# sevagh/umx.cpp

Hardware: AMD Instinct MI355X
Metric: realtime-factor (audio-sec/wall-sec) UMX-L 4-stem, 60 s seg (higher is better)
Workload: dtype f32 (activations as 2 x fp16 planes of the power-of-two-scaled row, integer weights exact in fp16, f32 accumulate on the fp16 matrix cores; fp32-grade: 1.4-2.2x the error of an fp32 evaluation, profiles/r06_v2_accuracy_vs_float64.txt)

## Files before the change

umx.cpp_amd/csrc/engine.hip:

```cpp
#include "../../include/umx_hip.h"
#include <chrono>
#include <dlfcn.h>

#include <algorithm>
#include <numeric>
#include <cmath>
#include <cstdio>
#include <cstdlib>
#include <cstring>
#include <map>
#include <mutex>
#include <string>
#include <vector>

#include "common.h"
#include "gemm_bf16x3.h"
#include "gemm_planes.h"
#include "gemm_planes_pp.h"
#include "gemm_planes_ps.h"
#include "lstm_kernels.h"
#include "lstm_batch.h"
#include "lstm_batch8.h"
#include "track_kernels.h"
#include "resample.h"
// ... 273 lines not shown
    int last = 0;
    for (const LstmKernel &k : kLstmKernels)
        if (k.family == family && k.hl != last)
        {
            s += (s.empty() ? "{" : ", ") + std::to_string(2 * k.hl);
            last = k.hl;
        }
    return s + "}";
}

struct GemmKernel
{
    const void *fn = nullptr;
    int lds = 0;
};

template <int MODE> static GemmKernel bx_kernel_m(int bq)
{
    if (bq == BQ_F32)
        return {kernel_ptr(gemm_bf16x3_kernel<MODE, BQ_F32>), BX_LDS_BYTES};
    if constexpr (MODE == G_FC1 || MODE == G_IH)
    {
        if (bq == BQ_U8X)
            return {kernel_ptr(gemm_bf16x3_kernel<MODE, BQ_U8X>), BX_LDS_BYTES};
        if (bq == BQ_U8)
            return {kernel_ptr(gemm_bf16x3_kernel<MODE, BQ_U8>), BX_LDS_BYTES};
    }
    else if (bq == BQ_U16)
        return {kernel_ptr(gemm_bf16x3_kernel<MODE, BQ_U16>), BX_LDS_BYTES};
    return {};
}
static GemmKernel bx_kernel(int mode, int bq)
{
    switch (mode)
    {
    case G_FC1: return bx_kernel_m<G_FC1>(bq);
    case G_IH: return bx_kernel_m<G_IH>(bq);
    case G_FC2: return bx_kernel_m<G_FC2>(bq);
    default: return bx_kernel_m<G_FC3>(bq);
    }
}

enum { GP_128 = 0, GP_256, GP_PP, GP_PS, GP_KINDS };
template <int MODE, int NBP> static GemmKernel gp_kernel_mn(int kind)
{
    switch (kind)
    {
    case GP_128: return {kernel_ptr(gemm_planes_kernel<MODE, NBP, 2, 2>), gp_lds_bytes(2, 2, NBP)};
    case GP_256: return {kernel_ptr(gemm_planes_kernel<MODE, NBP, 4, 4>), gp_lds_bytes(4, 4, NBP)};
    case GP_PP: return {kernel_ptr(gemm_planes_pp_kernel<MODE, NBP>), gp_lds_bytes(4, 4, NBP)};
    default: return {kernel_ptr(gemm_planes_ps_kernel<MODE, NBP>), ps_lds_bytes(NBP)};
    }
}
template <int MODE> static GemmKernel gp_kernel_m(int nbp, int kind)
{
    if constexpr (MODE == G_FC1 || MODE == G_IH)
    {
        if (nbp == 1)
            return gp_kernel_mn<MODE, 1>(kind);
    }
    return nbp == 2 ? gp_kernel_mn<MODE, 2>(kind) : GemmKernel{};
}
static GemmKernel gp_kernel(int mode, int nbp, int kind)
{
    switch (mode)
    {
    case G_FC1: return gp_kernel_m<G_FC1>(nbp, kind);
    case G_IH: return gp_kernel_m<G_IH>(nbp, kind);
    case G_FC2: return gp_kernel_m<G_FC2>(nbp, kind);
    default: return gp_kernel_m<G_FC3>(nbp, kind);
    }
}

struct umx_hip_ctx
{
    int device = 0, H = 0, Hl = 0, S = 0, N = 0, T = 0, Tp = 0, nbatch = 0;
    static constexpr int Mpad = 256;
    std::string err;
    std::vector<void *> allocs;
    TargetBufs tb[4];
    float *whh[3] = {}, *bhh[3] = {};
    float *window = nullptr, *nw = nullptr;
    float2 *tw1 = nullptr, *tw2 = nullptr;
    float *tap_tmp = nullptr;
    float *audio_in = nullptr, *out_dev[4] = {};
    static constexpr int kMaxSlots = 3;
    float *stage_in[kMaxSlots] = {}, *stage_out[kMaxSlots][4 * LSTMB_MAX_TRACKS] = {};
    int ensure_staging();
    hipEvent_t order_ev = nullptr;
    struct DeferredDownload
    {
        bool valid = false;
        int si = 0, nb = 0, n[LSTMB_MAX_TRACKS] = {};
        float *host[4 * LSTMB_MAX_TRACKS] = {};
    };
    int queue_download(const DeferredDownload &d, hipStream_t on);
    hipStream_t copy_stream = nullptr;
    float *state = nullptr, *state_alt = nullptr;
    Slot slot[kMaxSlots];
    int nslots = 2;
    int next_slot() const { return (int)(nseg % nslots); }
    void clear_used()
    {
        for (int si = 0; si < kMaxSlots; ++si)
            slot[si].used = false;
    }
    int B = 1;
    bool lstm_batched = false;
    unsigned tag_epoch = 0;
    unsigned next_tag_base()
    {
        tag_epoch = (tag_epoch + 1) & 0xFFFFF;
        return tag_epoch << 12;
    }
    int cur = 0;
    long long nseg = 0;
    size_t lsync_words = 0;
    bool persistent_ok = true;
    int n_cus = 256;
    struct PendingCall
    {
        int nb;
        const float *audio[LSTMB_MAX_TRACKS];
        int n[LSTMB_MAX_TRACKS];
        float *out[4 * LSTMB_MAX_TRACKS];
        float *host_out[4 * LSTMB_MAX_TRACKS];
        const float *host_audio[LSTMB_MAX_TRACKS];
        unsigned flags;
    };
    static constexpr int kBackupCalls = 8;
    std::vector<PendingCall> pending;
    bool pending_lost = false;
    float *backup = nullptr;
    bool no_recovery = false, recovering = false;
    int recover();
    int lstm_poll_delay = 0;
    int env_gemm_ps = -1;
    int env_gemm_pp = -1;
    const char *gemm_kernel_last[4] = {"none", "none", "none", "none"};
    const char *lstm_kernel_last = "none";
    int lstm_capacity = 0;
    unsigned last_flags = 0;
    hipStream_t stream = nullptr;

    void set_error(const std::string &s) { err = s; }

    template <class T_> int dalloc(T_ **p, size_t count, bool zero = true)
    {
        void *q = nullptr;
        UMX_HIP_CHECK(hipMalloc(&q, std::max<size_t>(count, 1) * sizeof(T_)));
        allocs.push_back(q);
        if (zero)
            UMX_HIP_CHECK(hipMemset(q, 0, std::max<size_t>(count, 1) * sizeof(T_)));
        *p = reinterpret_cast<T_ *>(q);
        return UMX_OK;
    }
    template <class T_> int upload(T_ **p, const std::vector<T_> &h)
    {
        int rc = dalloc(p, h.size(), false);
        if (rc)
            return rc;
        UMX_HIP_CHECK(hipMemcpy(*p, h.data(), h.size() * sizeof(T_), hipMemcpyHostToDevice));
        return UMX_OK;
    }
    int init(int device_, int hidden, int segment_samples, const umx_tensor_view *tensors, int n_tensors,
             unsigned create_flags, int n_tracks);
// ... 112 lines not shown
```

umx.cpp_amd/csrc/engine_init.h:

```cpp
namespace
{
bool dequant(const umx_tensor_view &tv, size_t expect, std::vector<float> &out)
{
    size_t nel = 1;
    for (int i = 0; i < tv.n_dims; ++i)
        nel *= (size_t)tv.ne[i];
    if (nel != expect)
        return false;
    out.resize(nel);
    if (tv.dtype == UMX_DTYPE_F32)
        memcpy(out.data(), tv.data, nel * sizeof(float));
    else if (tv.dtype == UMX_DTYPE_U8)
    {
        const uint8_t *q = static_cast<const uint8_t *>(tv.data);
        for (size_t i = 0; i < nel; ++i)
            out[i] = (float)q[i] * tv.scale + tv.offset;
    }
    else if (tv.dtype == UMX_DTYPE_U16)
    {
        const uint16_t *q = static_cast<const uint16_t *>(tv.data);
        for (size_t i = 0; i < nel; ++i)
            out[i] = (float)q[i] * tv.scale + tv.offset;
    }
    else
// ... 312 lines not shown
                std::vector<float> whhv, bih, bhhv;
                if ((!whh_all_u8 && !get(tg, "lstm.weight_hh" + sfx, (size_t)G * Hl, whhv)) ||
                    !get(tg, "lstm.bias_ih" + sfx, G, bih) || !get(tg, "lstm.bias_hh" + sfx, G, bhhv))
                    return UMX_ERR_MODEL;
                const int chain = tg * 2 + dir;
                const umx_tensor_view *hhv = view(tg, "lstm.weight_hh" + sfx);
                const unsigned char *hhq = whh_all_u8 ? static_cast<const unsigned char *>(hhv->data) : nullptr;
                if (whh_all_u8)
                {
                    whh_s[l][chain] = hhv->scale;
                    whh_o[l][chain] = hhv->offset;
                }
                for (int row = 0; row < G; ++row)
                {
                    const int sl = gate_row[row] / 64, col = gate_row[row] % 64;
                    ihb[(size_t)dir * G + gate_row[row]] = bih[row];
                    bhh_h[l][((size_t)chain * S + sl) * 64 + col] = bhhv[row];
                    for (int k = 0; k < Hl; ++k)
                    {
                        const size_t di = (((size_t)chain * S + sl) * Hl + k) * 64 + col;
                        if (whh_all_u8)
                            whh_qh[l][di] = hhq[(size_t)row * Hl + k];
                        else
                            whh_h[l][di] = whhv[(size_t)row * Hl + k];
                    }
                }
            }
            if (int rc = upload(&b.ih_b[l], ihb))
                return rc;
        }
    }
    for (int l = 0; l < 3; ++l)
    {
        if (whh_all_u8)
        {
            if (int rc = upload(&whh_q[l], whh_qh[l]))
                return rc;
            weight_bytes += whh_qh[l].size();
        }
        else
        {
            if (int rc = upload(&whh[l], whh_h[l]))
                return rc;
            weight_bytes += whh_h[l].size() * sizeof(float);
        }
        if (int rc = upload(&bhh[l], bhh_h[l]))
            return rc;
    }
    {
        std::vector<float> w(NFFT);
        static const float PI = 3.14159265359F;
        const float floatN = (float)(NFFT + 1);
        for (int n = 0; n < NFFT; ++n)
            w[n] = 0.5F * (1.0F - cosf(2.0F * PI * (float)n / (floatN - 1)));
        if (int rc = upload(&window, w))
            return rc;
        const size_t total = (size_t)NFFT + (size_t)HOP * (T - 1);
        std::vector<float> nwh(total, 0.f);
        for (int i = 0; i < T; ++i)
        {
            const size_t s0 = (size_t)i * HOP;
            for (size_t j = s0; j < std::min(total, s0 + NFFT); ++j)
                nwh[j] += w[j - s0] * w[j - s0];
        }
        if (int rc = upload(&nw, nwh))
            return rc;
        std::vector<float2> t1(256), t2(4096);
        for (int r = 0; r < 16; ++r)
            for (int k = 0; k < 16; ++k)
            {
                const double ph = -2.0 * M_PI * (double)(r * k) / 256.0;
                t1[r * 16 + k] = make_float2((float)cos(ph), (float)sin(ph));
            }
        for (int r = 0; r < 16; ++r)
            for (int j = 0; j < 256; ++j)
            {
                const double ph = -2.0 * M_PI * (double)(r * j) / 4096.0;
                t2[r * 256 + j] = make_float2((float)cos(ph), (float)sin(ph));
            }
        if (int rc = upload(&tw1, t1))
            return rc;
        if (int rc = upload(&tw2, t2))
            return rc;
    }
    if (int rc = dalloc(&audio_in, (size_t)2 * N))
        return rc;
    for (int k = 0; k < 4; ++k)
        if (int rc = dalloc(&out_dev[k], (size_t)2 * N))
            return rc;
    if (int rc = dalloc(&state, state_floats() * B))
        return rc;
    if (int rc = dalloc(&state_alt, state_floats() * B))
        return rc;
    if (int rc = dalloc(&backup, (size_t)kBackupCalls * 3 * state_floats() * B))
        return rc;
    lsync_words = LSTM_SYNC_HEADER_WORDS + std::max(granule_count(S) * 2, lstm_batched ? lstmb_granule_words(Hl) * ((B + LSTMB_GROUP_TRACKS - 1) / LSTMB_GROUP_TRACKS) : (size_t)0);
    nslots = 2;
    if (gemm_planes)
    {
        const unsigned long long rows = (unsigned long long)B * Tp + Mpad;
        const unsigned long long planes_bytes = 2ull * rows * (unsigned long long)std::max(KX, 2 * H) * 2ull;
        const unsigned long long mask_bytes = (unsigned long long)B * 2ull * T * MAGP * 4ull;
        if (planes_bytes >= (1ull << 31) || mask_bytes >= (1ull << 32))
        {
            set_error("track lanes x segment length exceed the 32-bit addressing of the plane GEMMs' operands: fewer lanes or a shorter segment");
            return UMX_ERR_ARG;
        }
    }
    for (int si = 0; si < nslots; ++si)
    {
        Slot &sl = slot[si];
        UMX_HIP_CHECK(hipStreamCreateWithFlags(&sl.stream, hipStreamNonBlocking));
        float *x_all = nullptr;
        if (int rc = dalloc(&x_all, ((size_t)B * Tp + Mpad) * KX))
            return rc;
        for (int tg = 0; tg < 4; ++tg)
        {
            float *cat_all = nullptr, *la_all = nullptr, *lb_all = nullptr, *P_all = nullptr, *a2_all = nullptr, *mag_all = nullptr;
            if (int rc = dalloc(&cat_all, ((size_t)B * Tp + Mpad) * 2 * H))
                return rc;
            if (int rc = dalloc(&la_all, ((size_t)B * Tp + Mpad) * H))
                return rc;
            if (int rc = dalloc(&lb_all, ((size_t)B * Tp + Mpad) * H))
                return rc;
            if (int rc = dalloc(&P_all, ((size_t)B * Tp + Mpad) * 4 * H))
                return rc;
            if (int rc = dalloc(&a2_all, ((size_t)B * Tp + Mpad) * H))
                return rc;
            if (int rc = dalloc(&mag_all, (size_t)B * 2 * T * MAGP))
                return rc;
            unsigned short *xs_p = nullptr, *cat_p = nullptr, *la_p = nullptr, *lb_p = nullptr, *a2_p = nullptr;
            float *rs[8] = {};
            if (gemm_planes)
            {
                if (int rc = dalloc(&xs_p, 2 * ((size_t)B * Tp + Mpad) * KX))
                    return rc;
                if (int rc = dalloc(&cat_p, 2 * ((size_t)B * Tp + Mpad) * 2 * H))
                    return rc;
                for (unsigned short **q : {&la_p, &lb_p, &a2_p})
                    if (int rc = dalloc(q, 2 * ((size_t)B * Tp + Mpad) * H))
                        return rc;
                for (int k = 0; k < 8; ++k)
                    if (int rc = dalloc(&rs[k], ((size_t)B * Tp + Mpad) * (k >= 2 && k <= 4 ? 2 : 1)))
                        return rc;
            }
            for (int ln = 0; ln < B; ++ln)
            {
                TargetAct &b = sl.lane[ln].ta[tg];
                b.cat = cat_all + (size_t)ln * Tp * 2 * H;
                b.la = la_all + (size_t)ln * Tp * H;
                b.lb = lb_all + (size_t)ln * Tp * H;
                b.P = P_all + (size_t)ln * Tp * 4 * H;
                b.a2 = a2_all + (size_t)ln * Tp * H;
                b.mag = mag_all + (size_t)ln * 2 * T * MAGP;
                if (gemm_planes)
                {
                    b.xs_p = xs_p + (size_t)ln * Tp * KX;
                    b.cat_p = cat_p + (size_t)ln * Tp * 2 * H;
                    b.la_p = la_p + (size_t)ln * Tp * H;
                    b.lb_p = lb_p + (size_t)ln * Tp * H;
                    b.a2_p = a2_p + (size_t)ln * Tp * H;
                    b.rs_xs = rs[0] + (size_t)ln * Tp;
                    b.rs_catL = rs[1] + (size_t)ln * Tp;
                    b.rs_catR = rs[2] + (size_t)ln * Tp;
                    b.rs_la = rs[3] + (size_t)ln * Tp;
                    b.rs_lb = rs[4] + (size_t)ln * Tp;
// ... 146 lines not shown
```

umx.cpp_amd/csrc/engine_stages.h:

```cpp
void umx_hip_ctx::launch_gemm(Lane &sl, hipStream_t st, int mode, int layer, const int *active, int nact, bool dbg)
{
    GemmArgs g;
    memset(&g, 0, sizeof g);
    g.M = Tp;
    g.T = T;
    int bq = BQ_F32;
    for (int i = 0; i < nact; ++i)
    {
        const TargetBufs &b = tb[active[i]];
        const TargetAct &c = sl.ta[active[i]];
        const GemmWeight &w = b.w[gemm_weight(mode, layer)];
        GemmTarget &t = g.t[i];
        switch (mode)
        {
        case G_FC1:
            t.A = sl.x; t.C = c.cat;
            t.e0 = b.bn1[0]; t.e1 = b.bn1[1]; t.e2 = b.bn1[2]; t.e3 = b.bn1[3];
            t.q0 = b.in_scale; t.q1 = b.in_mean;
            g.N = H; g.K = KX; g.lda = KX; g.ldc = 2 * H;
            break;
        case G_IH:
            t.A = layer == 0 ? c.cat : layer == 1 ? c.la : c.lb;
            t.C = c.P; t.e0 = b.ih_b[layer];
            g.N = 4 * H; g.K = H; g.lda = layer == 0 ? 2 * H : H; g.ldc = 4 * H;
// ... 306 lines not shown
        wm0.m[s] = L0.ta[s].mag;
    const int nchunk = (T + WIENER_CHUNK - 1) / WIENER_CHUNK;
    const int iters = (flags & UMX_FLAG_NO_WIENER) ? 1 : std::max(1, (int)((flags & UMX_FLAG_WIENER_ITERS_MASK) >> 16));
    if (iters > 1 && !sl.wv)
    {
        if ((unsigned long long)ls.v * sizeof(float) >= (1ull << 31))
        {
            set_error("Wiener EM iterations: the segment's PSD state exceeds the 32-bit addressing of the filter kernel: a shorter segment");
            return UMX_ERR_ARG;
        }
        if (int rc = dalloc(&sl.wv, (size_t)B * ls.v, false))
            return rc;
    }
    if (flags & UMX_FLAG_NO_WIENER)
    {
        if (!wiener_fused)
            for (int i = 0; i < lanes.count; ++i)
            {
                Lane &L = sl.lane[lanes.id[i]];
                WienerMags wm;
                for (int s = 0; s < 4; ++s)
                    wm.m[s] = L.ta[s].mag;
                const size_t nel = (size_t)2 * T * NBINS;
                hipLaunchKernelGGL(mixphase_kernel, dim3((unsigned)((nel + 255) / 256)), dim3(256), 0, st, L.spec, wm, T, L.y);
            }
    }
    else
    {
        hipLaunchKernelGGL(wiener_stats4_kernel<WIENER_STATS_NS>, dim3((NBINS + 63) / 64, nchunk * lanes.count, 4 / WIENER_STATS_NS), dim3(64), 0, st, L0.spec, wm0, T, L0.maxabs, L0.wpart, lanes, ls);
        hipLaunchKernelGGL(wiener_finish4_kernel, dim3(bt, 4, lanes.count), dim3(256), 0, st, L0.wpart, T, L0.Rc, lanes, ls);
        for (int it = 1; it < iters; ++it)
        {
            if (it == 1)
                hipLaunchKernelGGL(wiener_em_step_kernel<true>, dim3((NBINS + 63) / 64, nchunk * lanes.count), dim3(64), 0, st, L0.spec, wm0, sl.wv, T, L0.maxabs, L0.Rc, L0.wpart, lanes, ls);
            else
                hipLaunchKernelGGL(wiener_em_step_kernel<false>, dim3((NBINS + 63) / 64, nchunk * lanes.count), dim3(64), 0, st, L0.spec, wm0, sl.wv, T, L0.maxabs, L0.Rc, L0.wpart, lanes, ls);
            hipLaunchKernelGGL(wiener_finish4_kernel, dim3(bt, 4, lanes.count), dim3(256), 0, st, L0.wpart, T, L0.Rc, lanes, ls);
        }
        if (!wiener_fused)
            for (int i = 0; i < lanes.count; ++i)
            {
                const int ln = lanes.id[i];
                Lane &L = sl.lane[ln];
                WienerMags wm;
                for (int s = 0; s < 4; ++s)
                    wm.m[s] = L.ta[s].mag;
                if (iters > 1)
                    hipLaunchKernelGGL(wiener_apply_kernel<true>, dim3(bt, T), dim3(256), 0, st, L.spec, wm,
                                       reinterpret_cast<const float4 *>(sl.wv + (size_t)ln * ls.v), T, L.maxabs, L.Rc, L.y);
                else
                    hipLaunchKernelGGL(wiener_apply_kernel<false>, dim3(bt, T), dim3(256), 0, st, L.spec, wm, (const float4 *)nullptr, T, L.maxabs, L.Rc, L.y);
            }
    }
    OlaOut oo;
    oo.lanes = lanes;
    int nmax = 1;
    for (int i = 0; i < lanes.count; ++i)
    {
        const int ln = lanes.id[i];
        for (int s = 0; s < 4; ++s)
            oo.p[i][s] = out[4 * ln + s];
        oo.n[i] = n[ln];
        nmax = std::max(nmax, n[ln]);
    }
    stage_range(ST_ISTFT);
    UMX_HIP_CHECK(hipEventRecord(sl.ev[ST_ISTFT], st));
    if (!wiener_fused)
    {
        for (int i = 0; i < lanes.count; ++i)
        {
            Lane &L = sl.lane[lanes.id[i]];
            hipLaunchKernelGGL(istft_frames_kernel, dim3(T, 4), dim3(256), 0, st, L.y, T, window, nw, tw1, tw2, L.frames);
        }
    }
    else
    {
        float2 *ydbg = dbg ? L0.y : nullptr;
        if (sl.out_free_valid)
            UMX_HIP_CHECK(hipStreamWaitEvent(st, sl.out_free, 0));
        const int runs = std::max(1, std::min(T / 8, (4 * n_cus + lanes.count - 1) / lanes.count));
        const int run_len = std::max(3, (T + runs - 1) / runs), nruns = (T + run_len - 1) / run_len;
        if (flags & UMX_FLAG_NO_WIENER)
            hipLaunchKernelGGL((wiener_istft_kernel<false>), dim3(nruns, 1, lanes.count), dim3(1024), WI_LDS_BYTES, st, L0.spec, wm0,
                               T, L0.maxabs, L0.Rc, window, nw, tw1, tw2, L0.frames, ydbg, ls, run_len, oo);
        else if (iters > 1)
            hipLaunchKernelGGL(wiener_istft_v_kernel, dim3(nruns, 1, lanes.count), dim3(1024), WI_LDS_BYTES, st, (const float *)sl.wv, L0.spec, wm0,
                               T, L0.maxabs, L0.Rc, window, nw, tw1, tw2, L0.frames, ydbg, ls, run_len, oo);
        else
            hipLaunchKernelGGL((wiener_istft_kernel<true>), dim3(nruns, 1, lanes.count), dim3(1024), WI_LDS_BYTES, st, L0.spec, wm0,
                               T, L0.maxabs, L0.Rc, window, nw, tw1, tw2, L0.frames, ydbg, ls, run_len, oo);
        stage_range(ST_OLA);
        UMX_HIP_CHECK(hipEventRecord(sl.ev[ST_OLA], st));
        hipLaunchKernelGGL(wiener_ola_edges_kernel, dim3(3 * HOP / 256, nruns * 4, lanes.count), dim3(256), 0, st, L0.frames, ls.frames, T, run_len, oo);
    }
    if (!wiener_fused)
    {
        stage_range(ST_OLA);
        UMX_HIP_CHECK(hipEventRecord(sl.ev[ST_OLA], st));
        if (sl.out_free_valid)
            UMX_HIP_CHECK(hipStreamWaitEvent(st, sl.out_free, 0));
        hipLaunchKernelGGL(istft_ola_kernel, dim3((nmax + 255) / 256, 4, lanes.count), dim3(256), 0, st, L0.frames, ls.frames, T, oo);
    }
    stage_range(-1);
    UMX_HIP_CHECK(hipEventRecord(sl.ev[ST_COUNT], st));
    UMX_HIP_CHECK(hipGetLastError());
    sl.have_times = true;
    return UMX_OK;
}

int umx_hip_ctx::infer_device(const float *audio_dev, int n, float *const out[4], unsigned flags)
{
    if (!audio_dev)
    {
        set_error("infer_segment: need 1 <= n <= segment_samples and non-null audio");
        return UMX_ERR_ARG;
    }
    return infer_batch(1, &audio_dev, &n, out, flags);
}

int umx_hip_ctx::infer_batch(int nb, const float *const *audio_dev, const int *n, float *const *out, unsigned flags)
{
    StageRangeCloser close_ranges_on_return;
    if (nb < 1 || nb > B || !audio_dev || !n || !out)
    {
        set_error("infer: need 1 <= n_tracks <= the context's track count and non-null argument arrays");
        return UMX_ERR_ARG;
    }
    if (int rc = check_flags(flags))
        return rc;
    unsigned long long lane_mask = 0;
    for (int ln = 0; ln < nb; ++ln)
    {
        if (!audio_dev[ln])
            continue;
        if (n[ln] < 1 || n[ln] > N)
        {
            set_error("infer_segment: need 1 <= n <= segment_samples and non-null audio");
            return UMX_ERR_ARG;
        }
        for (int s = 0; s < 4; ++s)
            if (!out[4 * ln + s])
            {
                set_error("infer_segment: null output pointer");
                return UMX_ERR_ARG;
            }
        lane_mask |= 1ull << ln;
    }
    if (!lane_mask)
    {
        set_error("infer: no active track lane");
        return UMX_ERR_ARG;
    }
    if (ph_next != -1)
    {
        set_error("infer_segment: a phased segment is open (umx_hip_segment_end first)");
        return UMX_ERR_ARG;
    }
    UMX_HIP_CHECK(hipSetDevice(device));
    const int si = next_slot();
    Slot &sl = slot[si];
    Slot &prev = slot[(si + nslots - 1) % nslots];
    hipStream_t st = sl.stream;
    int active[4], nact;
    active_list(flags, active, nact);
    last_flags = flags;
    const size_t call_idx = pending_lost ? (size_t)kBackupCalls : pending.size();
    if (call_idx >= (size_t)kBackupCalls)
    {
        pending_lost = true;
        pending.clear();
    }
    else
    {
// ... 46 lines not shown
```

umx.cpp_amd/csrc/fft4096.h:

```cpp
#pragma once
#include "common.h"

namespace umx
{

constexpr int FFT_LDS_ELEMS = NFFT + NFFT / 16;

__device__ __forceinline__ int fft_pad(int i) { return i + (i >> 4); }

__device__ __forceinline__ float2 cmul(float2 a, float2 b)
{
    return make_float2(a.x * b.x - a.y * b.y, a.x * b.y + a.y * b.x);
}
__device__ __forceinline__ float2 cmul_tw(float2 a, float2 b)
{
    return make_float2(fmaf(a.x, b.x, -(a.y * b.y)), fmaf(a.x, b.y, a.y * b.x));
}
__device__ __forceinline__ float2 cadd(float2 a, float2 b) { return make_float2(a.x + b.x, a.y + b.y); }
__device__ __forceinline__ float2 csub(float2 a, float2 b) { return make_float2(a.x - b.x, a.y - b.y); }
__device__ __forceinline__ float2 cconj(float2 a) { return make_float2(a.x, -a.y); }

template <bool INV> __device__ __forceinline__ float2 mul_w4(float2 a)
{
    return INV ? make_float2(-a.y, a.x) : make_float2(a.y, -a.x);
}

template <bool INV> __device__ __forceinline__ void fft16(float2 (&v)[16])
{
    constexpr float C1 = 0.92387953251128674f;
    constexpr float S1 = 0.38268343236508977f;
    constexpr float R2 = 0.70710678118654752f;
    constexpr float SG = INV ? 1.0f : -1.0f;
    float2 a[4][4];
#pragma unroll
    for (int r0 = 0; r0 < 4; ++r0)
    {
        float2 x0 = v[r0], x1 = v[4 + r0], x2 = v[8 + r0], x3 = v[12 + r0];
        float2 s02 = cadd(x0, x2), d02 = csub(x0, x2), s13 = cadd(x1, x3), d13 = csub(x1, x3);
        float2 rot = mul_w4<INV>(d13);
        a[r0][0] = cadd(s02, s13);
        a[r0][1] = cadd(d02, rot);
        a[r0][2] = csub(s02, s13);
        a[r0][3] = csub(d02, rot);
    }
    const float2 w1 = make_float2(C1, SG * S1), w2 = make_float2(R2, SG * R2),
                 w3 = make_float2(S1, SG * C1), w6 = make_float2(-R2, SG * R2),
                 w9 = make_float2(-C1, -SG * S1);
    a[1][1] = cmul_tw(a[1][1], w1);
    a[1][2] = cmul_tw(a[1][2], w2);
    a[1][3] = cmul_tw(a[1][3], w3);
    a[2][1] = cmul_tw(a[2][1], w2);
    a[2][2] = mul_w4<INV>(a[2][2]);
    a[2][3] = cmul_tw(a[2][3], w6);
    a[3][1] = cmul_tw(a[3][1], w3);
    a[3][2] = cmul_tw(a[3][2], w6);
    a[3][3] = cmul_tw(a[3][3], w9);
#pragma unroll
    for (int q0 = 0; q0 < 4; ++q0)
    {
        float2 x0 = a[0][q0], x1 = a[1][q0], x2 = a[2][q0], x3 = a[3][q0];
        float2 s02 = cadd(x0, x2), d02 = csub(x0, x2), s13 = cadd(x1, x3), d13 = csub(x1, x3);
        float2 rot = mul_w4<INV>(d13);
        v[q0] = cadd(s02, s13);
        v[4 + q0] = cadd(d02, rot);
        v[8 + q0] = csub(s02, s13);
        v[12 + q0] = csub(d02, rot);
    }
}

template <bool INV, bool KEEP = false>
__device__ __forceinline__ void fft4096(float2 (&v)[16], float2 *buf, const float2 *__restrict__ tw1,
                                        const float2 *__restrict__ tw2, int j)
{
    fft16<INV>(v);
#pragma unroll
    for (int q = 0; q < 16; ++q)
        buf[fft_pad((j << 4) + q)] = v[q];
    __syncthreads();
    {
        const int k = j & 15;
#pragma unroll
        for (int r = 0; r < 16; ++r)
            v[r] = buf[fft_pad(j + 256 * r)];
        __syncthreads();
#pragma unroll
        for (int r = 1; r < 16; ++r)
        {
            float2 w = tw1[r * 16 + k];
            v[r] = cmul_tw(v[r], INV ? cconj(w) : w);
        }
        fft16<INV>(v);
        const int base = ((j - k) << 4) + k;
#pragma unroll
        for (int q = 0; q < 16; ++q)
            buf[fft_pad(base + 16 * q)] = v[q];
    }
    float2 w2[16];
#pragma unroll
    for (int r = 1; r < 16; ++r)
        w2[r] = tw2[r * 256 + j];
    __syncthreads();
    {
#pragma unroll
        for (int r = 0; r < 16; ++r)
            v[r] = buf[fft_pad(j + 256 * r)];
#pragma unroll
        for (int r = 1; r < 16; ++r)
        {
            const float2 w = w2[r];
            v[r] = cmul_tw(v[r], INV ? cconj(w) : w);
        }
        fft16<INV>(v);
        if (!KEEP)
#pragma unroll
            for (int q = 0; q < 16; ++q)
                buf[fft_pad(j + 256 * q)] = v[q];
    }
    if (!KEEP)
        __syncthreads();
}

template <bool INV>
__device__ __forceinline__ void fft4096(float2 (&v)[16], float2 *buf, const float2 *__restrict__ tw1,
                                        const float2 *__restrict__ tw2)
{
    fft4096<INV>(v, buf, tw1, tw2, (int)threadIdx.x);
}

}
```

umx.cpp_amd/csrc/wiener_istft.h:

```cpp
#pragma once
#include "stft_kernels.h"
#include "wiener_kernels.h"

#ifndef WI_PROFILE
#define WI_PROFILE 0
#endif

namespace umx
{

constexpr size_t WI_LDS_BYTES = (size_t)4 * FFT_LDS_ELEMS * sizeof(float2) + NFFT * sizeof(float) + HOP * sizeof(float) + 256 * sizeof(float2);

typedef float wi_f2 __attribute__((ext_vector_type(2)));
__device__ __forceinline__ float2 ld_stream(const float2 *p)
{
    const wi_f2 v = __builtin_nontemporal_load(reinterpret_cast<const wi_f2 *>(p));
    return make_float2(v.x, v.y);
}
__device__ __forceinline__ float ld_stream(const float *p) { return __builtin_nontemporal_load(p); }

typedef unsigned wi_u2 __attribute__((ext_vector_type(2)));
typedef unsigned wi_u4 __attribute__((ext_vector_type(4)));
template <int AUX> __device__ __forceinline__ float2 bld2(__amdgpu_buffer_rsrc_t rs, int voff, int soff)
{
    const wi_u2 v = __builtin_amdgcn_raw_buffer_load_b64(rs, voff, soff, AUX);
    return make_float2(__uint_as_float(v.x), __uint_as_float(v.y));
}
template <int AUX> __device__ __forceinline__ float bld1(__amdgpu_buffer_rsrc_t rs, int voff, int soff)
{
    return __uint_as_float(__builtin_amdgcn_raw_buffer_load_b32(rs, voff, soff, AUX));
}
template <int AUX> __device__ __forceinline__ float4 bld4(__amdgpu_buffer_rsrc_t rs, int voff, int soff)
{
    const wi_u4 v = __builtin_amdgcn_raw_buffer_load_b128(rs, voff, soff, AUX);
    return make_float4(__uint_as_float(v.x), __uint_as_float(v.y), __uint_as_float(v.z), __uint_as_float(v.w));
}
__device__ __forceinline__ void bst2(__amdgpu_buffer_rsrc_t rs, int voff, int soff, float2 v)
{
    const wi_u2 t = {__float_as_uint(v.x), __float_as_uint(v.y)};
    __builtin_amdgcn_raw_buffer_store_b64(t, rs, voff, soff, 0);
}

template <bool WIENER, bool VIN>
__device__ __forceinline__ void wiener_istft_run(const float2 *__restrict__ spec, WienerMags mags, const float *__restrict__ v, int T,
                                                                  const unsigned *__restrict__ maxabs_bits,
                                                                  const float *__restrict__ Rc, const float *__restrict__ window,
                                                                  const float *__restrict__ nw, const float2 *__restrict__ tw1,
                                                                  const float2 *__restrict__ tw2, float2 *__restrict__ frames,
                                                                  float2 *__restrict__ y_dbg, WienerStrides ls, int run_len, OlaOut out)
{
    static_assert(WIENER || !VIN, "the PSDs of the filter");
    extern __shared__ __attribute__((aligned(16))) float2 wi_buf[];
    float *const wi_win = reinterpret_cast<float *>(wi_buf + 4 * FFT_LDS_ELEMS);
    float *const wi_nwp = wi_win + NFFT;
    float2 *const wi_tw1 = reinterpret_cast<float2 *>(wi_nwp + HOP);
    constexpr int NSRC = 4, WI_THREADS = 256 * NSRC;
    const LaneSet &lanes = out.lanes;
    {
        const int ln = lanes.id[blockIdx.z];
        spec += (size_t)ln * ls.spec;
        Rc += (size_t)ln * ls.rc;
        frames += (size_t)ln * ls.frames;
        maxabs_bits += ln;
        if (y_dbg)
            y_dbg += (size_t)ln * ls.y;
        if (VIN)
            v += (size_t)ln * ls.v;
#pragma unroll
        for (int s = 0; s < 4; ++s)
            mags.m[s] += (size_t)ln * ls.mag;
    }
    constexpr int src0 = 0;
    const int tid = threadIdx.x;
#pragma unroll
    for (int r = 0; r < 4; ++r)
        wi_win[tid + 1024 * r] = window[tid + 1024 * r];
    wi_nwp[tid] = nw[3 * HOP + tid];
    if (tid < 256)
        wi_tw1[tid] = tw1[tid];
    const __amdgpu_buffer_rsrc_t rs_spec = __builtin_amdgcn_make_buffer_rsrc(const_cast<float2 *>(spec), 0, (int)((size_t)2 * T * NBINS * 8), 0x00020000);
    __amdgpu_buffer_rsrc_t rs_mag[4];
#pragma unroll
    for (int s = 0; s < 4; ++s)
        rs_mag[s] = __builtin_amdgcn_make_buffer_rsrc(const_cast<float *>(mags.m[s]), 0, (int)((size_t)2 * T * MAGP * 4), 0x00020000);
    const __amdgpu_buffer_rsrc_t rs_v = __builtin_amdgcn_make_buffer_rsrc(const_cast<float *>(v), 0, (int)((size_t)T * NBINS * 16), 0x00020000);
    const __amdgpu_buffer_rsrc_t rs_rc = __builtin_amdgcn_make_buffer_rsrc(const_cast<float *>(Rc), 0, (int)((size_t)4 * NBINS * 16), 0x00020000);
    const __amdgpu_buffer_rsrc_t rs_nw = __builtin_amdgcn_make_buffer_rsrc(const_cast<float *>(nw), 0, (int)(((size_t)(T - 1) * HOP + NFFT) * 4), 0x00020000);
    const float max_abs = WIENER ? wiener_max_abs(maxabs_bits) : 1.0f, rmax = 1.0f / max_abs;
    const int f0 = (int)blockIdx.x * run_len, f1 = min(T, f0 + run_len);
    const int g = __builtin_amdgcn_readfirstlane(tid >> 8);
    float2 *const stem = reinterpret_cast<float2 *>(out.p[blockIdx.z][src0 + g]);
    const int n_out = out.n[blockIdx.z];
    const __amdgpu_buffer_rsrc_t rs_stem = __builtin_amdgcn_make_buffer_rsrc(stem, 0, n_out * 8, 0x00020000);
    [[maybe_unused]] long long pf[5] = {0, 0, 0, 0, 0};
    float2 open[3][4];
#pragma unroll
    for (int c = 0; c < 3; ++c)
#pragma unroll
        for (int q = 0; q < 4; ++q)
            open[c][q] = make_float2(0.f, 0.f);
    float2 Xq[2][2];
    float mq[2][2][4];
#define WI_REQUEST(f_, tl_, q_)                                                                                                        \
    {                                                                                                                                  \
        Xq[q_][0] = bld2<2>(rs_spec, (tl_) * 8, ((0 * T + (f_)) * NBINS + WI_THREADS * (q_)) * 8);                                      \
        Xq[q_][1] = bld2<2>(rs_spec, (tl_) * 8, ((1 * T + (f_)) * NBINS + WI_THREADS * (q_)) * 8);                                      \
        if (VIN)                                                                                                                       \
        {                                                                                                                              \
            const float4 vf_ = bld4<2>(rs_v, (tl_) * 16, ((f_) * NBINS + WI_THREADS * (q_)) * 16);                                      \
            mq[q_][0][0] = vf_.x;                                                                                                      \
            mq[q_][0][1] = vf_.y;                                                                                                      \
            mq[q_][0][2] = vf_.z;                                                                                                      \
            mq[q_][0][3] = vf_.w;                                                                                                      \
        }                                                                                                                              \
        else                                                                                                                           \
            _Pragma("unroll") for (int s = 0; s < 4; ++s)                                                                              \
            {                                                                                                                          \
                mq[q_][0][s] = bld1<2>(rs_mag[s], (tl_) * 4, ((0 * T + (f_)) * MAGP + WI_THREADS * (q_)) * 4);  \
                mq[q_][1][s] = bld1<2>(rs_mag[s], (tl_) * 4, ((1 * T + (f_)) * MAGP + WI_THREADS * (q_)) * 4);                          \
            }                                                                                                                          \
    }
    if (f0 < f1)
    {
        int tl0 = tid;
        asm volatile("" : "+v"(tl0));
        WI_REQUEST(f0, tl0, 0);
    }
    for (int f = f0; f < f1; ++f)
    {
    [[maybe_unused]] long long c0 = 0, c1 = 0, c2 = 0, c3 = 0, c4 = 0;
    if (WI_PROFILE)
        c0 = clock64();
    int tl = tid;
    asm volatile("" : "+v"(tl));
    const int j = tl & 255;
    float4 rc0[4];
    if (WIENER)
    {
#pragma unroll
        for (int s = 0; s < 4; ++s)
            rc0[s] = bld4<0>(rs_rc, tl * 16, (s * NBINS) * 16);
        __builtin_amdgcn_sched_barrier(0);
    }
    WI_REQUEST(f, tl, 1);
    constexpr int NQ = (NFFT / 2 + WI_THREADS) / WI_THREADS;
#pragma unroll
    for (int q = 0; q < NQ; ++q)
    {
        const int b = tl + WI_THREADS * q;
        if (b > NFFT / 2)
            break;
        float2 X0, X1;
        float m0[4], m1[4];
        if (q < 2)
        {
            X0 = Xq[q < 2 ? q : 0][0];
            X1 = Xq[q < 2 ? q : 0][1];
#pragma unroll
            for (int s = 0; s < 4; ++s)
            {
                m0[s] = mq[q < 2 ? q : 0][0][s];
                m1[s] = VIN ? 0.f : mq[q < 2 ? q : 0][1][s];
            }
        }
        else
        {
            X0 = bld2<2>(rs_spec, tl * 8, ((0 * T + f) * NBINS + WI_THREADS * q) * 8);
            X1 = bld2<2>(rs_spec, tl * 8, ((1 * T + f) * NBINS + WI_THREADS * q) * 8);
            if (VIN)
            {
                const float4 vf = bld4<2>(rs_v, tl * 16, (f * NBINS + WI_THREADS * q) * 16);
                m0[0] = vf.x;
                m0[1] = vf.y;
                m0[2] = vf.z;
                m0[3] = vf.w;
            }
            else
#pragma unroll
                for (int s = 0; s < 4; ++s)
                {
                    m0[s] = bld1<2>(rs_mag[s], tl * 4, ((0 * T + f) * MAGP + WI_THREADS * q) * 4);
                    m1[s] = bld1<2>(rs_mag[s], tl * 4, ((1 * T + f) * MAGP + WI_THREADS * q) * 4);
                }
        }
        if (!VIN)
        {
            const float h0 = mix_magnitude(X0), h1 = mix_magnitude(X1);
#pragma unroll
            for (int s = 0; s < 4; ++s)
            {
                m0[s] *= h0;
                m1[s] *= h1;
            }
        }
        WienerBin wb;
        float4 rc[4];
        float2 p0, p1;
        if (WIENER)
        {
#pragma unroll
            for (int s = 0; s < 4; ++s)
                rc[s] = q == 0 ? rc0[s] : bld4<0>(rs_rc, tl * 16, (s * NBINS + WI_THREADS * q) * 16);
            if (VIN)
                wiener_bin_setup_v(X0, X1, m0, rc, max_abs, rmax, wb);
            else
                wiener_bin_setup(X0, X1, m0, m1, rc, max_abs, rmax, wb);
        }
        else
        {
            p0 = unit_phasor(X0);
            p1 = unit_phasor(X1);
        }
#pragma unroll
        for (int sl = 0; sl < NSRC; ++sl)
        {
            const int s = src0 + sl;
            float2 o[2];
            if (WIENER)
                wiener_bin_apply(wb, s, rc[sl], max_abs, o);
            else
            {
                const float ms0 = m0[sl], ms1 = m1[sl];
                o[0] = make_float2(ms0 * p0.x, ms0 * p0.y);
                o[1] = make_float2(ms1 * p1.x, ms1 * p1.y);
            }
            if (y_dbg)
            {
                y_dbg[(((size_t)s * 2 + 0) * T + f) * NBINS + b] = o[0];
                y_dbg[(((size_t)s * 2 + 1) * T + f) * NBINS + b] = o[1];
            }
            float2 a = o[0], bb = o[1];
            if (b == 0 || b == NFFT / 2)
            {
                a.y = 0.f;
                bb.y = 0.f;
            }
            float2 *buf = wi_buf + sl * FFT_LDS_ELEMS;
            buf[fft_pad(b)] = make_float2(a.x - bb.y, a.y + bb.x);
            if (b > 0 && b < NFFT / 2)
                buf[fft_pad(NFFT - b)] = make_float2(a.x + bb.y, bb.x - a.y);
        }
    }
    if (WI_PROFILE)
        c1 = clock64();
    __syncthreads();
    if (WI_PROFILE)
        c2 = clock64();
    float2 *buf = wi_buf + g * FFT_LDS_ELEMS;
    float2 v[16];
#pragma unroll
    for (int r = 0; r < 16; ++r)
        v[r] = buf[fft_pad(j + 256 * r)];
    __syncthreads();
    fft4096<true, true>(v, buf, wi_tw1, tw2, j);
    if (WI_PROFILE)
        c3 = clock64();
    float2 *dst = frames + ((size_t)(src0 + g) * T + f) * NFFT;
    const int start = f * HOP;
    const bool keep = f - f0 < 3;
    const bool interior = f >= 3 && f + 3 <= T - 1;
    auto overlap_add = [&](auto in_c) {
        constexpr bool IN = decltype(in_c)::value;
        float d4[4] = {0.f, 0.f, 0.f, 0.f}, r4[4] = {0.f, 0.f, 0.f, 0.f};
        if (IN)
        {
#pragma unroll
            for (int q = 0; q < 4; ++q)
            {
                d4[q] = wi_nwp[j + 256 * q] + 1e-8f;
                r4[q] = __builtin_amdgcn_rcpf(d4[q]);
            }
            if (f + 1 < f1)
            {
                WI_REQUEST(f + 1, tl, 0);
            }
            __builtin_amdgcn_sched_barrier(0);
        }
#pragma unroll
        for (int r = 0; r < 16; ++r)
        {
            const int i = j + 256 * r;
            const float2 z = v[r];
            const float w = wi_win[i];
            const float den = IN ? d4[r & 3] : bld1<0>(rs_nw, j * 4, (start + 256 * r) * 4) + 1e-8f;
            const float rden = IN ? r4[r & 3] : __builtin_amdgcn_rcpf(den);
            const float2 val = make_float2(div_by(z.x * w * 1.0f / float(NFFT), den, rden), div_by(z.y * w * 1.0f / float(NFFT), den, rden));
            if (keep)
                dst[i] = val;
            const int c = r >> 2, q = r & 3;
            const float2 a = c < 3 ? open[c < 3 ? c : 0][q] : make_float2(0.f, 0.f);
            const float2 sum = make_float2(a.x + val.x, a.y + val.y);
            if (c == 0)
            {
                if (f >= f0 + 3)
                    bst2(rs_stem, j * 8, (start + 256 * r - NFFT / 2) * 8, sum);
            }
            else
                open[c - 1][q] = sum;
        }
        if (!IN && f + 1 < f1)
        {
            WI_REQUEST(f + 1, tl, 0);
        }
    };
    if (interior)
        overlap_add(std::true_type{});
    else
        overlap_add(std::false_type{});
    asm volatile("s_waitcnt lgkmcnt(0)\n\ts_barrier" ::: "memory");
    if (WI_PROFILE)
    {
        c4 = clock64();
        pf[0] += c1 - c0;
        pf[1] += c2 - c1;
        pf[2] += c3 - c2;
        pf[3] += c4 - c3;
    }
    }
    {
        const int j = tid & 255;
#pragma unroll
        for (int c = 0; c < 3; ++c)
#pragma unroll
            for (int q = 0; q < 4; ++q)
            {
                const int h = f1 + c, s_out = h * HOP + j + 256 * q - NFFT / 2;
                if (h >= f0 + 3 && s_out >= 0 && s_out < n_out)
                    stem[s_out] = open[c][q];
            }
    }
#undef WI_REQUEST
    if (WI_PROFILE && blockIdx.x == 7 && blockIdx.z == 3 && (tid == 0 || tid == 777))
        printf("# wiener_istft thread %d, %d frames: cycles per frame  loads+gains %lld  barrier %lld  transform %lld  weight+overlap-add+drain %lld\n", tid,
               f1 - f0, pf[0] / (f1 - f0), pf[1] / (f1 - f0), pf[2] / (f1 - f0), pf[3] / (f1 - f0));
}

#define WI_PARAMS                                                                                                                  \
    const float2 *__restrict__ spec, WienerMags mags, int T, const unsigned *__restrict__ maxabs_bits, const float *__restrict__ Rc,         \
        const float *__restrict__ window, const float *__restrict__ nw, const float2 *__restrict__ tw1, const float2 *__restrict__ tw2,     \
        float2 *__restrict__ frames, float2 *__restrict__ y_dbg, WienerStrides ls, int run_len, OlaOut out
template <bool WIENER> __global__ __launch_bounds__(1024) void wiener_istft_kernel(WI_PARAMS)
{
    wiener_istft_run<WIENER, false>(spec, mags, nullptr, T, maxabs_bits, Rc, window, nw, tw1, tw2, frames, y_dbg, ls, run_len, out);
}
__global__ __launch_bounds__(1024) void wiener_istft_v_kernel(const float *__restrict__ v, WI_PARAMS)
{
    wiener_istft_run<true, true>(spec, mags, v, T, maxabs_bits, Rc, window, nw, tw1, tw2, frames, y_dbg, ls, run_len, out);
}
#undef WI_PARAMS

__global__ __launch_bounds__(256) void wiener_ola_edges_kernel(const float2 *__restrict__ frames, size_t frames_stride, int T, int run_len, OlaOut out)
{
    const int run = blockIdx.y >> 2, src = blockIdx.y & 3;
    const int f0 = run * run_len, h = f0 + (int)(blockIdx.x * 256 + threadIdx.x) / HOP, k = (int)(blockIdx.x * 256 + threadIdx.x) % HOP;
    const int s_out = h * HOP + k - NFFT / 2, n_out = out.n[blockIdx.z];
    if (f0 >= T || s_out < 0 || s_out >= n_out)
        return;
    frames += (size_t)out.lanes.id[blockIdx.z] * frames_stride;
    float2 *const stem = reinterpret_cast<float2 *>(out.p[blockIdx.z][src]);
    const int fa = max(0, h - 3), fb = min(T - 1, h);
    float2 acc = fa < f0 ? stem[s_out] : make_float2(0.f, 0.f);
    for (int f = max(fa, f0); f <= fb; ++f)
    {
        const float2 c = frames[((size_t)src * T + f) * NFFT + (h - f) * HOP + k];
        acc.x += c.x;
        acc.y += c.y;
    }
    stem[s_out] = acc;
}

}
```

Baseline: 36920.

## Vectorize Wiener-iSTFT loads with paired bins and packed twiddles; split the prefetch

Each thread in the fused Wiener/iSTFT kernel now handles two adjacent frequency bins (2*tl, 2*tl+1) instead of bins strided by 1024. This lets the spectrum, magnitude, v and Rc reads become wider 8- and 16-byte loads. The second-stage FFT twiddles are repacked on the host as float4 pairs, so each thread issues half as many global loads for them. The next-frame prefetch is split into two halves: the second half is issued in the middle of the overlap-add loop to spread memory traffic, and a clamped frame index replaces the branch. The cost is more register pressure from wider prefetch buffers, plus one redundant prefetch on the last frame.

New measurement: 37180, median of 6. Within noise of the previous version (+0.7%).

```diff
diff --git a/umx.cpp_amd/csrc/engine.hip b/umx.cpp_amd/csrc/engine.hip
--- a/umx.cpp_amd/csrc/engine.hip
+++ b/umx.cpp_amd/csrc/engine.hip
@@ -379,6 +379,7 @@
     float *whh[3] = {}, *bhh[3] = {};
     float *window = nullptr, *nw = nullptr;
     float2 *tw1 = nullptr, *tw2 = nullptr;
+    float4 *tw2p = nullptr;
     float *tap_tmp = nullptr;
     float *audio_in = nullptr, *out_dev[4] = {};
     static constexpr int kMaxSlots = 3;
diff --git a/umx.cpp_amd/csrc/engine_init.h b/umx.cpp_amd/csrc/engine_init.h
--- a/umx.cpp_amd/csrc/engine_init.h
+++ b/umx.cpp_amd/csrc/engine_init.h
@@ -418,6 +418,15 @@
             return rc;
         if (int rc = upload(&tw2, t2))
             return rc;
+        std::vector<float4> t2p(2048);
+        for (int k = 0; k < 8; ++k)
+            for (int j = 0; j < 256; ++j)
+            {
+                const float2 a = t2[(2 * k) * 256 + j], b = t2[(2 * k + 1) * 256 + j];
+                t2p[k * 256 + j] = make_float4(a.x, a.y, b.x, b.y);
+            }
+        if (int rc = upload(&tw2p, t2p))
+            return rc;
     }
     if (int rc = dalloc(&audio_in, (size_t)2 * N))
         return rc;
diff --git a/umx.cpp_amd/csrc/engine_stages.h b/umx.cpp_amd/csrc/engine_stages.h
--- a/umx.cpp_amd/csrc/engine_stages.h
+++ b/umx.cpp_amd/csrc/engine_stages.h
@@ -412,13 +412,13 @@
         const int run_len = std::max(3, (T + runs - 1) / runs), nruns = (T + run_len - 1) / run_len;
         if (flags & UMX_FLAG_NO_WIENER)
             hipLaunchKernelGGL((wiener_istft_kernel<false>), dim3(nruns, 1, lanes.count), dim3(1024), WI_LDS_BYTES, st, L0.spec, wm0,
-                               T, L0.maxabs, L0.Rc, window, nw, tw1, tw2, L0.frames, ydbg, ls, run_len, oo);
+                               T, L0.maxabs, L0.Rc, window, nw, tw1, tw2p, L0.frames, ydbg, ls, run_len, oo);
         else if (iters > 1)
             hipLaunchKernelGGL(wiener_istft_v_kernel, dim3(nruns, 1, lanes.count), dim3(1024), WI_LDS_BYTES, st, (const float *)sl.wv, L0.spec, wm0,
-                               T, L0.maxabs, L0.Rc, window, nw, tw1, tw2, L0.frames, ydbg, ls, run_len, oo);
+                               T, L0.maxabs, L0.Rc, window, nw, tw1, tw2p, L0.frames, ydbg, ls, run_len, oo);
         else
             hipLaunchKernelGGL((wiener_istft_kernel<true>), dim3(nruns, 1, lanes.count), dim3(1024), WI_LDS_BYTES, st, L0.spec, wm0,
-                               T, L0.maxabs, L0.Rc, window, nw, tw1, tw2, L0.frames, ydbg, ls, run_len, oo);
+                               T, L0.maxabs, L0.Rc, window, nw, tw1, tw2p, L0.frames, ydbg, ls, run_len, oo);
         stage_range(ST_OLA);
         UMX_HIP_CHECK(hipEventRecord(sl.ev[ST_OLA], st));
         hipLaunchKernelGGL(wiener_ola_edges_kernel, dim3(3 * HOP / 256, nruns * 4, lanes.count), dim3(256), 0, st, L0.frames, ls.frames, T, run_len, oo);
diff --git a/umx.cpp_amd/csrc/fft4096.h b/umx.cpp_amd/csrc/fft4096.h
--- a/umx.cpp_amd/csrc/fft4096.h
+++ b/umx.cpp_amd/csrc/fft4096.h
@@ -68,7 +68,7 @@
     }
 }
 
-template <bool INV, bool KEEP = false>
+template <bool INV, bool KEEP = false, bool TW2_PAIRS = false>
 __device__ __forceinline__ void fft4096(float2 (&v)[16], float2 *buf, const float2 *__restrict__ tw1,
                                         const float2 *__restrict__ tw2, int j)
 {
@@ -96,9 +96,20 @@
             buf[fft_pad(base + 16 * q)] = v[q];
     }
     float2 w2[16];
+    if (TW2_PAIRS)
+    {
 #pragma unroll
-    for (int r = 1; r < 16; ++r)
-        w2[r] = tw2[r * 256 + j];
+        for (int k = 0; k < 8; ++k)
+        {
+            const float4 t = reinterpret_cast<const float4 *>(tw2)[k * 256 + j];
+            w2[2 * k] = make_float2(t.x, t.y);
+            w2[2 * k + 1] = make_float2(t.z, t.w);
+        }
+    }
+    else
+#pragma unroll
+        for (int r = 1; r < 16; ++r)
+            w2[r] = tw2[r * 256 + j];
     __syncthreads();
     {
 #pragma unroll
diff --git a/umx.cpp_amd/csrc/wiener_istft.h b/umx.cpp_amd/csrc/wiener_istft.h
--- a/umx.cpp_amd/csrc/wiener_istft.h
+++ b/umx.cpp_amd/csrc/wiener_istft.h
@@ -46,7 +46,7 @@
                                                                   const unsigned *__restrict__ maxabs_bits,
                                                                   const float *__restrict__ Rc, const float *__restrict__ window,
                                                                   const float *__restrict__ nw, const float2 *__restrict__ tw1,
-                                                                  const float2 *__restrict__ tw2, float2 *__restrict__ frames,
+                                                                  const float4 *__restrict__ tw2p, float2 *__restrict__ frames,
                                                                   float2 *__restrict__ y_dbg, WienerStrides ls, int run_len, OlaOut out)
 {
     static_assert(WIENER || !VIN, "the PSDs of the filter");
@@ -54,7 +54,7 @@
     float *const wi_win = reinterpret_cast<float *>(wi_buf + 4 * FFT_LDS_ELEMS);
     float *const wi_nwp = wi_win + NFFT;
     float2 *const wi_tw1 = reinterpret_cast<float2 *>(wi_nwp + HOP);
-    constexpr int NSRC = 4, WI_THREADS = 256 * NSRC;
+    constexpr int NSRC = 4;
     const LaneSet &lanes = out.lanes;
     {
         const int ln = lanes.id[blockIdx.z];
@@ -99,32 +99,39 @@
 #pragma unroll
         for (int q = 0; q < 4; ++q)
             open[c][q] = make_float2(0.f, 0.f);
-    float2 Xq[2][2];
-    float mq[2][2][4];
-#define WI_REQUEST(f_, tl_, q_)                                                                                                        \
+    float4 Xp[2];
+    float2 mp[2][4];
+#define WI_REQUEST_A(f_, tl_)                                                                                                          \
     {                                                                                                                                  \
-        Xq[q_][0] = bld2<2>(rs_spec, (tl_) * 8, ((0 * T + (f_)) * NBINS + WI_THREADS * (q_)) * 8);                                      \
-        Xq[q_][1] = bld2<2>(rs_spec, (tl_) * 8, ((1 * T + (f_)) * NBINS + WI_THREADS * (q_)) * 8);                                      \
+        Xp[0] = bld4<2>(rs_spec, (tl_) * 16, ((0 * T + (f_)) * NBINS) * 8);                                                             \
+        Xp[1] = bld4<2>(rs_spec, (tl_) * 16, ((1 * T + (f_)) * NBINS) * 8);                                                             \
+        if (!VIN)                                                                                                                      \
+            _Pragma("unroll") for (int s = 0; s < 2; ++s)                                                                              \
+                mp[0][s] = bld2<2>(rs_mag[s], (tl_) * 8, ((0 * T + (f_)) * MAGP) * 4);                       \
+    }
+#define WI_REQUEST_B(f_, tl_)                                                                                                          \
+    {                                                                                                                                  \
         if (VIN)                                                                                                                       \
+            _Pragma("unroll") for (int e = 0; e < 2; ++e)                                                                              \
+            {                                                                                                                          \
+                const float4 vf_ = bld4<2>(rs_v, (tl_) * 32, ((f_) * NBINS + e) * 16);                                                  \
+                mp[e][0] = make_float2(vf_.x, vf_.y);                                                                                  \
+                mp[e][1] = make_float2(vf_.z, vf_.w);                                                                                  \
+            }                                                                                                                          \
+        else                                                                                                                           \
         {                                                                                                                              \
-            const float4 vf_ = bld4<2>(rs_v, (tl_) * 16, ((f_) * NBINS + WI_THREADS * (q_)) * 16);                                      \
-            mq[q_][0][0] = vf_.x;                                                                                                      \
-            mq[q_][0][1] = vf_.y;                                                                                                      \
-            mq[q_][0][2] = vf_.z;                                                                                                      \
-            mq[q_][0][3] = vf_.w;                                                                                                      \
+            _Pragma("unroll") for (int s = 2; s < 4; ++s)                                                                              \
+                mp[0][s] = bld2<2>(rs_mag[s], (tl_) * 8, ((0 * T + (f_)) * MAGP) * 4);                                                  \
+            _Pragma("unroll") for (int s = 0; s < 4; ++s)                                                                              \
+                mp[1][s] = bld2<2>(rs_mag[s], (tl_) * 8, ((1 * T + (f_)) * MAGP) * 4);                                                  \
         }                                                                                                                              \
-        else                                                                                                                           \
-            _Pragma("unroll") for (int s = 0; s < 4; ++s)                                                                              \
-            {                                                                                                                          \
-                mq[q_][0][s] = bld1<2>(rs_mag[s], (tl_) * 4, ((0 * T + (f_)) * MAGP + WI_THREADS * (q_)) * 4);  \
-                mq[q_][1][s] = bld1<2>(rs_mag[s], (tl_) * 4, ((1 * T + (f_)) * MAGP + WI_THREADS * (q_)) * 4);                          \
-            }                                                                                                                          \
     }
     if (f0 < f1)
     {
         int tl0 = tid;
         asm volatile("" : "+v"(tl0));
-        WI_REQUEST(f0, tl0, 0);
+        WI_REQUEST_A(f0, tl0);
+        WI_REQUEST_B(f0, tl0);
     }
     for (int f = f0; f < f1; ++f)
     {
@@ -139,37 +146,44 @@
     {
 #pragma unroll
         for (int s = 0; s < 4; ++s)
-            rc0[s] = bld4<0>(rs_rc, tl * 16, (s * NBINS) * 16);
+            rc0[s] = bld4<0>(rs_rc, tl * 32, (s * NBINS) * 16);
         __builtin_amdgcn_sched_barrier(0);
     }
-    WI_REQUEST(f, tl, 1);
-    constexpr int NQ = (NFFT / 2 + WI_THREADS) / WI_THREADS;
-#pragma unroll
-    for (int q = 0; q < NQ; ++q)
-    {
-        const int b = tl + WI_THREADS * q;
-        if (b > NFFT / 2)
+#pragma unroll
+    for (int q = 0; q < 3; ++q)
+    {
+        if (q == 2 && tl != 0)
             break;
+        const int b = q < 2 ? 2 * tl + q : NFFT / 2;
         float2 X0, X1;
         float m0[4], m1[4];
         if (q < 2)
         {
-            X0 = Xq[q < 2 ? q : 0][0];
-            X1 = Xq[q < 2 ? q : 0][1];
+            X0 = q == 0 ? make_float2(Xp[0].x, Xp[0].y) : make_float2(Xp[0].z, Xp[0].w);
+            X1 = q == 0 ? make_float2(Xp[1].x, Xp[1].y) : make_float2(Xp[1].z, Xp[1].w);
 #pragma unroll
             for (int s = 0; s < 4; ++s)
             {
-                m0[s] = mq[q < 2 ? q : 0][0][s];
-                m1[s] = VIN ? 0.f : mq[q < 2 ? q : 0][1][s];
+                if (VIN)
+                {
+                    const float2 h = mp[q < 2 ? q : 0][s >> 1];
+                    m0[s] = (s & 1) ? h.y : h.x;
+                    m1[s] = 0.f;
+                }
+                else
+                {
+                    m0[s] = q == 0 ? mp[0][s].x : mp[0][s].y;
+                    m1[s] = q == 0 ? mp[1][s].x : mp[1][s].y;
+                }
             }
         }
         else
         {
-            X0 = bld2<2>(rs_spec, tl * 8, ((0 * T + f) * NBINS + WI_THREADS * q) * 8);
-            X1 = bld2<2>(rs_spec, tl * 8, ((1 * T + f) * NBINS + WI_THREADS * q) * 8);
+            X0 = bld2<2>(rs_spec, 0, ((0 * T + f) * NBINS + NFFT / 2) * 8);
+            X1 = bld2<2>(rs_spec, 0, ((1 * T + f) * NBINS + NFFT / 2) * 8);
             if (VIN)
             {
-                const float4 vf = bld4<2>(rs_v, tl * 16, (f * NBINS + WI_THREADS * q) * 16);
+                const float4 vf = bld4<2>(rs_v, 0, (f * NBINS + NFFT / 2) * 16);
                 m0[0] = vf.x;
                 m0[1] = vf.y;
                 m0[2] = vf.z;
@@ -179,8 +193,8 @@
 #pragma unroll
                 for (int s = 0; s < 4; ++s)
                 {
-                    m0[s] = bld1<2>(rs_mag[s], tl * 4, ((0 * T + f) * MAGP + WI_THREADS * q) * 4);
-                    m1[s] = bld1<2>(rs_mag[s], tl * 4, ((1 * T + f) * MAGP + WI_THREADS * q) * 4);
+                    m0[s] = bld1<2>(rs_mag[s], 0, ((0 * T + f) * MAGP + NFFT / 2) * 4);
+                    m1[s] = bld1<2>(rs_mag[s], 0, ((1 * T + f) * MAGP + NFFT / 2) * 4);
                 }
         }
         if (!VIN)
@@ -200,7 +214,7 @@
         {
 #pragma unroll
             for (int s = 0; s < 4; ++s)
-                rc[s] = q == 0 ? rc0[s] : bld4<0>(rs_rc, tl * 16, (s * NBINS + WI_THREADS * q) * 16);
+                rc[s] = q == 0 ? rc0[s] : bld4<0>(rs_rc, q == 1 ? tl * 32 : 0, (s * NBINS + (q == 1 ? 1 : NFFT / 2)) * 16);
             if (VIN)
                 wiener_bin_setup_v(X0, X1, m0, rc, max_abs, rmax, wb);
             else
@@ -252,13 +266,14 @@
     for (int r = 0; r < 16; ++r)
         v[r] = buf[fft_pad(j + 256 * r)];
     __syncthreads();
-    fft4096<true, true>(v, buf, wi_tw1, tw2, j);
+    fft4096<true, true, true>(v, buf, wi_tw1, reinterpret_cast<const float2 *>(tw2p), j);
     if (WI_PROFILE)
         c3 = clock64();
     float2 *dst = frames + ((size_t)(src0 + g) * T + f) * NFFT;
     const int start = f * HOP;
     const bool keep = f - f0 < 3;
     const bool interior = f >= 3 && f + 3 <= T - 1;
+    const int fn = min(f + 1, f1 - 1);
     auto overlap_add = [&](auto in_c) {
         constexpr bool IN = decltype(in_c)::value;
         float d4[4] = {0.f, 0.f, 0.f, 0.f}, r4[4] = {0.f, 0.f, 0.f, 0.f};
@@ -270,15 +285,18 @@
                 d4[q] = wi_nwp[j + 256 * q] + 1e-8f;
                 r4[q] = __builtin_amdgcn_rcpf(d4[q]);
             }
-            if (f + 1 < f1)
-            {
-                WI_REQUEST(f + 1, tl, 0);
-            }
+            WI_REQUEST_A(fn, tl);
             __builtin_amdgcn_sched_barrier(0);
         }
 #pragma unroll
         for (int r = 0; r < 16; ++r)
         {
+            if (IN && r == 8)
+            {
+                __builtin_amdgcn_sched_barrier(0);
+                WI_REQUEST_B(fn, tl);
+                __builtin_amdgcn_sched_barrier(0);
+            }
             const int i = j + 256 * r;
             const float2 z = v[r];
             const float w = wi_win[i];
@@ -298,9 +316,10 @@
             else
                 open[c - 1][q] = sum;
         }
-        if (!IN && f + 1 < f1)
-        {
-            WI_REQUEST(f + 1, tl, 0);
+        if (!IN)
+        {
+            WI_REQUEST_A(fn, tl);
+            WI_REQUEST_B(fn, tl);
         }
     };
     if (interior)
@@ -329,7 +348,8 @@
                     stem[s_out] = open[c][q];
             }
     }
-#undef WI_REQUEST
+#undef WI_REQUEST_A
+#undef WI_REQUEST_B
     if (WI_PROFILE && blockIdx.x == 7 && blockIdx.z == 3 && (tid == 0 || tid == 777))
         printf("# wiener_istft thread %d, %d frames: cycles per frame  loads+gains %lld  barrier %lld  transform %lld  weight+overlap-add+drain %lld\n", tid,
                f1 - f0, pf[0] / (f1 - f0), pf[1] / (f1 - f0), pf[2] / (f1 - f0), pf[3] / (f1 - f0));
@@ -337,15 +357,15 @@
 
 #define WI_PARAMS                                                                                                                  \
     const float2 *__restrict__ spec, WienerMags mags, int T, const unsigned *__restrict__ maxabs_bits, const float *__restrict__ Rc,         \
-        const float *__restrict__ window, const float *__restrict__ nw, const float2 *__restrict__ tw1, const float2 *__restrict__ tw2,     \
+        const float *__restrict__ window, const float *__restrict__ nw, const float2 *__restrict__ tw1, const float4 *__restrict__ tw2p,     \
         float2 *__restrict__ frames, float2 *__restrict__ y_dbg, WienerStrides ls, int run_len, OlaOut out
 template <bool WIENER> __global__ __launch_bounds__(1024) void wiener_istft_kernel(WI_PARAMS)
 {
-    wiener_istft_run<WIENER, false>(spec, mags, nullptr, T, maxabs_bits, Rc, window, nw, tw1, tw2, frames, y_dbg, ls, run_len, out);
+    wiener_istft_run<WIENER, false>(spec, mags, nullptr, T, maxabs_bits, Rc, window, nw, tw1, tw2p, frames, y_dbg, ls, run_len, out);
 }
 __global__ __launch_bounds__(1024) void wiener_istft_v_kernel(const float *__restrict__ v, WI_PARAMS)
 {
-    wiener_istft_run<true, true>(spec, mags, v, T, maxabs_bits, Rc, window, nw, tw1, tw2, frames, y_dbg, ls, run_len, out);
+    wiener_istft_run<true, true>(spec, mags, v, T, maxabs_bits, Rc, window, nw, tw1, tw2p, frames, y_dbg, ls, run_len, out);
 }
 #undef WI_PARAMS
 
```
